# Alxaline/BraTS21

Hardware: AMD Instinct MI355X
Metric: train patches/sec (4x128^3, width-48) (higher is better)
Workload: dtype bf16; 1 GPU; equiunet width=48, batch=2/GPU of 4x128^3 synthetic patches, fwd + deep-supervision Dice + bwd + ranger (BASELINE.json configs[1]); global_batch=2, parallelism=dp1

## Files before the change

### brats21_amd/csrc/common.hpp

```cpp
#pragma once
#include <hip/hip_runtime.h>
#include <stdint.h>
#include <stdio.h>
#include <atomic>
#include <type_traits>
#include "../../include/brats_hip.h"

typedef uint16_t bf16_t;
#ifdef BRATS_FP16
typedef __attribute__((ext_vector_type(8))) _Float16 bf16x8;
typedef __attribute__((ext_vector_type(4))) _Float16 bf16x4;
#else
typedef __attribute__((ext_vector_type(8))) __bf16 bf16x8;
typedef __attribute__((ext_vector_type(4))) __bf16 bf16x4;
#endif
typedef __attribute__((ext_vector_type(4))) float f32x4;
typedef __attribute__((ext_vector_type(2))) float f32x2;
typedef __attribute__((ext_vector_type(4))) uint32_t u32x4;
typedef __attribute__((ext_vector_type(2))) uint32_t u32x2;

#define DEVI __device__ __forceinline__

#ifdef BRATS_FP16
DEVI float bf2f(bf16_t v) { return (float)__builtin_bit_cast(_Float16, v); }
// ... 190 lines not shown

static inline int ceil_div(int a, int b) { return (a + b - 1) / b; }

static inline int device_cus() {
  static int ncu = 0;
  if (!ncu) {
    int dev = 0;
    hipDeviceProp_t prop;
    ncu = (hipGetDevice(&dev) == hipSuccess && hipGetDeviceProperties(&prop, dev) == hipSuccess) ? prop.multiProcessorCount : 256;
  }
  return ncu;
}

template <typename T> struct type_tag { using type = T; };
template <typename F> static inline auto with_flag(bool on, F&& f) {
  if (on) return f(std::true_type{});
  return f(std::false_type{});
}
template <typename F> static inline auto with_storage(int dtype, F&& f) {
  if (dtype == BRATS_BF16) return f(type_tag<bf16_t>{});
  return f(type_tag<float>{});
}
template <typename F> static inline auto with_stream(int dtype, bool nt, F&& f) {
  return with_storage(dtype, [&](auto t) { return with_flag(nt, [&](auto n) { return f(t, n); }); });
}
template <typename F> static inline auto with_stream16(int dtype, bool nt, F&& f) {
  if (dtype != BRATS_BF16) return f(type_tag<float>{}, std::false_type{});
  return with_flag(nt, [&](auto n) { return f(type_tag<bf16_t>{}, n); });
}
template <typename F> static inline auto with_act_stream(int dtype, bool heavy, bool nt, F&& f) {
  if (heavy) return with_storage(dtype, [&](auto t) { return f(t, std::true_type{}, std::false_type{}); });
  return with_stream(dtype, nt, [&](auto t, auto n) { return f(t, std::false_type{}, n); });
}

static inline bool big_tensor(int dtype, size_t elems) { return stream_nt(elems * (dtype == BRATS_BF16 ? 2 : 4)); }
static inline bool big_tensor16(int dtype, size_t elems) { return dtype == BRATS_BF16 && stream_nt(elems * 2); }

static inline int vec_width(int dtype) { return dtype == BRATS_BF16 ? 8 : 4; }

static inline int stream_grid(size_t total, int block, int cap) {
  size_t b = (total + block - 1) / block;
  return (int)(b < 1 ? 1 : (b > (size_t)cap ? (size_t)cap : b));
}

struct Walk {
  int cv, vl;
  size_t blocks;
  unsigned grid(size_t cap) const { return (unsigned)(blocks < 1 ? 1 : (blocks > cap ? cap : blocks)); }
};
static inline Walk voxel_walk(int vw, int voxels, int C) {
  const int cv = C / vw, vl = 256 / cv;
  return Walk{cv, vl, ((size_t)voxels + (size_t)vl * 8 - 1) / ((size_t)vl * 8)};
}
```

### brats21_amd/csrc/gen_twin_dispatch.py

```python
#!/usr/bin/env python3
import re
import sys

BOTH = {"brats_conv3d_set_vs8", "brats_conv3d_set_kp", "brats_conv3d_set_wgrad_alltaps", "brats_conv3d_set_x3_wgrad_fused",
        "brats_upsample_bwd_set_fused"}
DATA = {"brats_conv3d_f8_fwd", "brats_conv3d_wgrad_f8", "brats_conv3d_pack_weights_multi"}

txt = re.sub(r"/\*.*?\*/", " ", open(sys.argv[1]).read(), flags=re.S)
protos = {}
for m in re.finditer(r"(const char\s*\*|size_t|int)\s+(brats_[a-z0-9_]+)\s*\(([^)]*)\)\s*;", txt):
    protos[m.group(2)] = (" ".join(m.group(1).split()), " ".join(m.group(3).split()))
names = []
for path in sys.argv[2:]:
    for m in re.finditer(r'extern "C" [a-z_ \*]+?BRATS_API\((brats_[a-z0-9_]+)\)\(', open(path).read()):
        names.append(m.group(1))
print("// GENERATED by gen_twin_dispatch.py from include/brats_hip.h -- do not edit")
print('#include "../../include/brats_hip.h"')
print('extern "C" {')
for n in names:
    if n not in protos:
        raise SystemExit(f"{n} is defined in a twinned translation unit but not declared in brats_hip.h")
    ret, args = protos[n]
    arglist = [] if args in ("", "void") else [a.strip() for a in args.split(",")]
    argnames = [re.search(r"([A-Za-z_][A-Za-z0-9_]*)$", a).group(1) for a in arglist]
    call = ", ".join(argnames)
    sig = args if arglist else "void"
    print(f"{ret} {n}_bf16({sig});")
    print(f"{ret} {n}_f16({sig});")
    if n in DATA:
        if n + "_f16" not in protos:
            raise SystemExit(f"{n}_f16 must be declared in brats_hip.h (16-bit data, no dtype argument)")
        print(f"{ret} {n}({sig}) {{ return {n}_bf16({call}); }}")
    elif n in BOTH:
        print(f"{ret} {n}({sig}) {{ {n}_f16({call}); return {n}_bf16({call}); }}")
    elif "dtype" in argnames:
        call16 = ", ".join("BRATS_BF16" if a == "dtype" else a for a in argnames)
        callx3 = ", ".join("BRATS_X3_BF16" if a == "dtype" else a for a in argnames)
        print(f"{ret} {n}({sig}) {{ return dtype == BRATS_F16 ? {n}_f16({call16}) : dtype == BRATS_X3_F16 ? {n}_f16({callx3}) : {n}_bf16({call}); }}")
    else:
        print(f"{ret} {n}({sig}) {{ return {n}_bf16({call}); }}")
print("}")
```

### brats21_amd/csrc/norm.hip

```cpp
#include "twin_begin.hpp"
#include "common.hpp"

#include "se.hpp"

constexpr int GN_MAX_SPLITS = 64;
__global__ void gn_chan_reduce_kernel(const float* __restrict__ stats, int tps, int C, double* __restrict__ part) {
  const int n = blockIdx.y, c0 = blockIdx.x * 16;
  const int cl = threadIdx.x & 15, tl = threadIdx.x >> 4;
  const int c = c0 + cl;
  const int per = (tps + gridDim.z - 1) / gridDim.z;
  const int t0 = blockIdx.z * per, t1 = min(tps, t0 + per);
  double s1 = 0.0, s2 = 0.0;
  if (c < C) {
    for (int t = t0 + tl; t < t1; t += 16) {
      const f32x2 v = *(const f32x2*)(stats + (((size_t)n * tps + t) * C + c) * 2);
      s1 += v[0];
      s2 += v[1];
    }
  }
  __shared__ double r1[256], r2[256];
  r1[threadIdx.x] = s1;
  r2[threadIdx.x] = s2;
  __syncthreads();
  for (int m = 128; m >= 16; m >>= 1) {
// ... 265 lines not shown
  if (!HEAVY && act == BRATS_ACT_RELU) run(std::true_type{});
  else run(std::false_type{});
  if (amax) record_absmax<T>(mx, amax);
}

extern "C" int BRATS_API(brats_affine_act_fwd)(const void* y, int ypitch, const float* scale_shift, void* z, int zpitch,
                                    int dtype, int act, float slope_value, const float* slope_dev, int N, int voxels, int C,
                                    float* amax, brats_stream_t s) {
  const SlopeArg slope{slope_value, slope_dev};
  const int vw = vec_width(dtype);
  if (!y || !z || !scale_shift || C % vw || ypitch % vw || zpitch % vw || C / vw > 256)
    BRATS_FAIL(BRATS_E_ARG, "affine_act_fwd: C and pitches must be multiples of %d (C <= %d)", vw, 256 * vw);
  const bool big = big_tensor(dtype, (size_t)N * voxels * C);
  dim3 grid(voxel_walk(vw, voxels, C).grid(big ? 8192 : 2048), N);
  with_act_stream(dtype, act > BRATS_ACT_LEAKY, big, [&](auto t, auto heavy, auto nt) {
    using T = typename decltype(t)::type;
    hipLaunchKernelGGL((affine_act_kernel<T, decltype(heavy)::value, decltype(nt)::value>), grid, dim3(256), 0, (hipStream_t)s, (const T*)y,
                       ypitch, scale_shift, (T*)z, zpitch, act, slope, voxels, C, (uint32_t*)amax);
  });
  BRATS_CHECK_LAUNCH();
  return 0;
}

template <typename T> struct Raw16;
template <> struct Raw16<bf16_t> {
  typedef u32x4 type;
  template <bool NT> static DEVI type load(const bf16_t* p) {
    if constexpr (NT) return __builtin_nontemporal_load((const u32x4*)p); else return *(const u32x4*)p;
  }
  static DEVI void unpack(const type& v, float* o) {
#pragma unroll
    for (int i = 0; i < 4; ++i) unpack2(v[i], o[2 * i], o[2 * i + 1]);
  }
};
template <> struct Raw16<float> {
  typedef f32x4 type;
  template <bool NT> static DEVI type load(const float* p) { return *(const f32x4*)p; }
  static DEVI void unpack(const type& v, float* o) { o[0] = v[0]; o[1] = v[1]; o[2] = v[2]; o[3] = v[3]; }
};

template <typename T, bool NT = false, bool AM = false>
__global__ void __launch_bounds__(256) affine_act_pool_kernel(const T* __restrict__ y, int ypitch, const float* __restrict__ scale_shift,
                                                              T* __restrict__ z, int zpitch, T* __restrict__ p, int ppitch, int act,
                                                              SlopeArg sl, int D, int H, int W, int C, int with_avg,
                                                              uint32_t* __restrict__ amax, uint8_t* __restrict__ argmax) {
  constexpr int VW = 16 / sizeof(T);
  typedef typename Raw16<T>::type raw_t;
  extern __shared__ __attribute__((aligned(16))) char pool_lds[];
  raw_t* xch = (raw_t*)pool_lds;
  const float slope = sl.p ? *sl.p : sl.v;
  const bool relu = act == BRATS_ACT_RELU;
  const int n = blockIdx.y;
  const int cv = C / VW;
  int xb = (blockDim.x / cv) & ~1;
  if (xb > W) xb = W;
  const int mycv = threadIdx.x % cv, myvl = threadIdx.x / cv, c0 = mycv * VW;
  const bool lane_on = myvl < xb;
  const int Do = D / 2, Ho = H / 2, Wo = W / 2;
  const int segs = (W + xb - 1) / xb;
  const size_t items = (size_t)Do * Ho * segs, voxels = (size_t)D * H * W;
  float sc[VW], sh[VW];
#pragma unroll
  for (int j = 0; j < VW; ++j) {
    sc[j] = lane_on ? scale_shift[((size_t)n * C + c0 + j) * 2] : 0.f;
    sh[j] = lane_on ? scale_shift[((size_t)n * C + c0 + j) * 2 + 1] : 0.f;
  }
  const T* yb = y + (size_t)n * voxels * ypitch + c0;
  T* zb = z + (size_t)n * voxels * zpitch + c0;
  T* pb = p + (size_t)n * Do * Ho * Wo * ppitch + c0;
  float amx = 0.f;
  int buf = 0;
  for (size_t item = blockIdx.x; item < items; item += gridDim.x, buf ^= 1) {
    const int seg = (int)(item % segs);
    const size_t rp = item / segs;
    const int yo = (int)(rp % Ho), zo = (int)(rp / Ho);
    const int x = seg * xb + myvl;
    const bool on = lane_on && x < W;
    raw_t mine[4];
    if (on) {
      raw_t raw[4];
      size_t vox[4];
#pragma unroll
      for (int k = 0; k < 4; ++k) {
        vox[k] = ((size_t)(2 * zo + (k >> 1)) * H + (2 * yo + (k & 1))) * W + x;
        raw[k] = Raw16<T>::template load<NT>(yb + vox[k] * ypitch);
      }
#pragma unroll
      for (int k = 0; k < 4; ++k) {
        float a[VW];
        Raw16<T>::unpack(raw[k], a);
#pragma unroll
        for (int j = 0; j < VW; ++j) {
          const float pre = a[j] * sc[j] + sh[j];
          const float neg = relu ? 0.f : pre * slope;
          a[j] = pre > 0.f ? pre : neg;
        }
        vstore<T, VW, NT>(zb + vox[k] * zpitch, a);
        if constexpr (std::is_same<T, float>::value) {
          mine[k] = raw_t{a[0], a[1], a[2], a[3]};
        } else {
#pragma unroll
          for (int q = 0; q < 4; ++q) mine[k][q] = pack2(a[2 * q], a[2 * q + 1]);
        }
        if (amax) {
          float r[VW];
          Raw16<T>::unpack(mine[k], r);
#pragma unroll
          for (int j = 0; j < VW; ++j) amx = __builtin_fmaxf(amx, __builtin_fabsf(r[j]));
        }
        xch[((size_t)buf * blockDim.x + threadIdx.x) * 4 + k] = mine[k];
      }
    }
    __syncthreads();
    if (on && !(myvl & 1)) {
      float mx[VW], sm[VW];
      int am[VW];
#pragma unroll
      for (int j = 0; j < VW; ++j) { mx[j] = -INFINITY; sm[j] = 0.f; am[j] = 0; }
#pragma unroll
      for (int k = 0; k < 4; ++k) {
        float a[VW], b[VW];
        Raw16<T>::unpack(mine[k], a);
        Raw16<T>::unpack(xch[((size_t)buf * blockDim.x + threadIdx.x + cv) * 4 + k], b);
#pragma unroll
        for (int j = 0; j < VW; ++j) {
          if constexpr (AM) {
            if (a[j] > mx[j] || a[j] != a[j]) { mx[j] = a[j]; am[j] = 2 * k; }
            if (b[j] > mx[j] || b[j] != b[j]) { mx[j] = b[j]; am[j] = 2 * k + 1; }
          } else {
            mx[j] = (a[j] > mx[j] || a[j] != a[j]) ? a[j] : mx[j];
            mx[j] = (b[j] > mx[j] || b[j] != b[j]) ? b[j] : mx[j];
          }
          sm[j] = (sm[j] + a[j]) + b[j];
        }
      }
      const size_t pvox = ((size_t)zo * Ho + yo) * Wo + (x >> 1);
      T* po = pb + pvox * ppitch;
      if constexpr (AM) {
        uint32_t w[VW / 4];
#pragma unroll
        for (int q = 0; q < VW / 4; ++q) w[q] = am[4 * q] | (am[4 * q + 1] << 8) | (am[4 * q + 2] << 16) | (am[4 * q + 3] << 24);
        uint32_t* ap = (uint32_t*)(argmax + ((size_t)n * Do * Ho * Wo + pvox) * C + c0);
#pragma unroll
        for (int q = 0; q < VW / 4; ++q) ap[q] = w[q];
      }
      Vec<T, VW>::store(po, mx);
      if (with_avg) {
#pragma unroll
        for (int j = 0; j < VW; ++j) sm[j] *= 0.125f;
        Vec<T, VW>::store(po + C, sm);
      }
    }
  }
  if (amax) record_absmax<T>(amx, amax);
}

extern "C" int BRATS_API(brats_affine_act_pool_fwd)(const void* y, int ypitch, const float* scale_shift, void* z, int zpitch, void* pooled,
                                         int ppitch, unsigned char* argmax, int dtype, int act, float slope_value,
                                         const float* slope_dev, int N, int D, int H, int W, int C, int with_avg, float* amax,
                                         brats_stream_t s) {
  const SlopeArg slope{slope_value, slope_dev};
  const int vw = vec_width(dtype);
  if (!y || !z || !pooled || !scale_shift || C % vw || ypitch % vw || zpitch % vw || ppitch % vw || C / vw > 256 || ((D | H | W) & 1))
    BRATS_FAIL(BRATS_E_ARG, "affine_act_pool_fwd: C / pitches multiples of %d (C <= %d), even spatial dims", vw, 256 * vw);
  if (act > BRATS_ACT_LEAKY) BRATS_FAIL(BRATS_E_UNSUPPORTED, "affine_act_pool_fwd: relu / leakyrelu only (act=%d)", act);
  int xb = (256 / (C / vw)) & ~1;
  if (xb < 2) BRATS_FAIL(BRATS_E_UNSUPPORTED, "affine_act_pool_fwd: C=%d leaves no pooling pair per block", C);
  if (xb > W) xb = W;
  const size_t items = (size_t)(D / 2) * (H / 2) * ((W + xb - 1) / xb);
  const bool big = big_tensor16(dtype, (size_t)N * D * H * W * C);
  dim3 grid(stream_grid(items, 1, big ? 8192 : 2048), N);
  const size_t lds = (size_t)2 * 256 * 4 * 16;
  with_stream16(dtype, big, [&](auto t, auto nt) {
    with_flag(argmax != nullptr, [&](auto am) {
      using T = typename decltype(t)::type;
      hipLaunchKernelGGL((affine_act_pool_kernel<T, decltype(nt)::value, decltype(am)::value>), grid, dim3(256), lds, (hipStream_t)s,
                         (const T*)y, ypitch, scale_shift, (T*)z, zpitch, (T*)pooled, ppitch, act, slope, D, H, W, C, with_avg,
                         (uint32_t*)amax, argmax);
    });
  });
  BRATS_CHECK_LAUNCH();
  return 0;
}

template <int VW, typename F>
DEVI void lane_reduce_plane(float* scr, const float* a, bool live, int myvl, int vl_n, int C, int c0, F&& put) {
  __syncthreads();
  if (live) {
#pragma unroll
    for (int j = 0; j < VW; ++j) scr[myvl * C + c0 + j] = a[j];
  }
  __syncthreads();
  for (int c = threadIdx.x; c < C; c += blockDim.x) {
    float t = 0.f;
    for (int l = 0; l < vl_n; ++l) t += scr[l * C + c];
    put(c, t);
  }
}

struct HeadFold {
  const float* dl = nullptr;
  const float* w = nullptr;
  float* hpart = nullptr;
  const void* dskip = nullptr;
  const void* dpool = nullptr;
  const uint8_t* argmax = nullptr;
  int dskip_pitch = 0, dpool_pitch = 0, D = 0, H = 0, W = 0;
  int with_avg = 0;
};
template <typename T, int VW>
DEVI void pool_dz(const HeadFold& hf, int n, size_t vox, int c0, int C, typename Raw16<T>::type& skr, typename Raw16<T>::type& dpr,
                  typename Raw16<T>::type& avr, uint32_t (&aw)[VW / 4], int& kk) {
  const int x = (int)(vox % hf.W);
  const size_t t = vox / hf.W;
  const int yy = (int)(t % hf.H), z = (int)(t / hf.H);
  const size_t pvox = (((size_t)n * (hf.D / 2) + (z >> 1)) * (hf.H / 2) + (yy >> 1)) * (hf.W / 2) + (x >> 1);
  kk = ((z & 1) << 2) | ((yy & 1) << 1) | (x & 1);
  skr = Raw16<T>::template load<false>((const T*)hf.dskip + ((size_t)n * hf.D * hf.H * hf.W + vox) * hf.dskip_pitch + c0);
  dpr = Raw16<T>::template load<false>((const T*)hf.dpool + pvox * hf.dpool_pitch + c0);
  if (hf.with_avg) avr = Raw16<T>::template load<false>((const T*)hf.dpool + pvox * hf.dpool_pitch + C + c0);
  else avr = dpr;
#pragma unroll
  for (int q = 0; q < VW / 4; ++q) aw[q] = ((const uint32_t*)(hf.argmax + pvox * C + c0))[q];
}
// ... 1486 lines not shown
```

### brats21_amd/csrc/pool_up.hip

```cpp
#include "twin_begin.hpp"
#include "common.hpp"

constexpr int POOL_MAX_BLOCKS = 8192;

template <typename T>
__global__ void maxpool2_fwd_kernel(const T* __restrict__ x, int xpitch, T* __restrict__ y, int ypitch, int N, int C,
                                    int D, int H, int W, int with_avg, uint8_t* __restrict__ argmax) {
  constexpr int VW = 16 / sizeof(T);
  const int cv = C / VW, Do = D / 2, Ho = H / 2, Wo = W / 2;
  const size_t total = (size_t)N * Do * Ho * Wo * cv;
  for (size_t it = (size_t)blockIdx.x * blockDim.x + threadIdx.x; it < total; it += (size_t)gridDim.x * blockDim.x) {
    const int c0 = (int)(it % cv) * VW;
    size_t v = it / cv;
    const int xo = v % Wo; v /= Wo;
    const int yo = v % Ho; v /= Ho;
    const int zo = v % Do;
    const int n = (int)(v / Do);
    float mx[VW], sm[VW];
    int am[VW];
#pragma unroll
    for (int j = 0; j < VW; ++j) { mx[j] = -INFINITY; sm[j] = 0.f; am[j] = 0; }
#pragma unroll
    for (int k = 0; k < 8; ++k) {
      const int z = 2 * zo + (k >> 2), yy = 2 * yo + ((k >> 1) & 1), xx = 2 * xo + (k & 1);
// ... 284 lines not shown
#pragma unroll
    for (int a = 0; a < 2; ++a)
#pragma unroll
      for (int b = 0; b < 4; ++b)
#pragma unroll
        for (int j = 0; j < V2; ++j) o[a][b][j] = f2{0.f, 0.f};
#pragma unroll
    for (int pz = 0; pz < 3; ++pz) {
      const int zi = zb + pz < D ? zb + pz : D - 1;
      f2 t[4][V2];
#pragma unroll
      for (int b = 0; b < 4; ++b)
#pragma unroll
        for (int j = 0; j < V2; ++j) t[b][j] = f2{0.f, 0.f};
#pragma unroll
      for (int r = 0; r < 4; ++r) {
        const int yi = yb + r < H ? yb + r : H - 1;
        float v0[VW], v1[VW];
        if constexpr (LDSX) {
          const T* row = (const T*)up_lds + (size_t)(pz * 4 + r) * W * C + c0;
          Vec<T, VW>::load(row + (size_t)lx.i0 * C, v0);
          Vec<T, VW>::load(row + (size_t)lx.i1 * C, v1);
        } else {
          const T* row = xb + (size_t)(zi * H + yi) * W * xpitch + c0;
          Vec<T, VW>::load(row + (size_t)lx.i0 * xpitch, v0);
          Vec<T, VW>::load(row + (size_t)lx.i1 * xpitch, v1);
        }
#pragma unroll
        for (int j = 0; j < V2; ++j) {
          const f2 xl = fma2(lx.w1, f2{v1[2 * j], v1[2 * j + 1]}, lx.w0 * f2{v0[2 * j], v0[2 * j + 1]});
#pragma unroll
          for (int b = 0; b < 4; ++b) t[b][j] = fma2(wy[b][r], xl, t[b][j]);
        }
      }
#pragma unroll
      for (int a = 0; a < 2; ++a)
#pragma unroll
        for (int b = 0; b < 4; ++b)
#pragma unroll
          for (int j = 0; j < V2; ++j) o[a][b][j] = fma2(wz[a][pz], t[b][j], o[a][b][j]);
    }
#pragma unroll
    for (int a = 0; a < 2; ++a)
#pragma unroll
      for (int b = 0; b < 4; ++b) {
        float of[VW];
#pragma unroll
        for (int j = 0; j < V2; ++j) { of[2 * j] = o[a][b][j][0]; of[2 * j + 1] = o[a][b][j][1]; }
        vstore<T, VW, NT>(yb_ + ((size_t)((zo0 + a) * Ho + yo0 + b) * Wo + xo) * ypitch + c0, of);
      }
  }
}

extern "C" int BRATS_API(brats_upsample_fwd)(const void* x, int xpitch, void* y, int ypitch, int dtype, int N, int C, int D, int H,
                                  int W, int scale, brats_stream_t s) {
  const int vw = vec_width(dtype);
  if (!x || !y || C % vw || xpitch % vw || ypitch % vw || scale < 1)
    BRATS_FAIL(BRATS_E_ARG, "upsample_fwd: C/pitch must be multiples of %d", vw);
  const size_t rows = (size_t)N * D * scale * H * scale;
  const unsigned grid = (unsigned)(rows > 65536 ? 65536 : rows);
  const float sd = ac_scale(D, D * scale), sh = ac_scale(H, H * scale), sw = ac_scale(W, W * scale);
  if (scale == 2 && H % 2 == 0 && N <= 65535 && D <= 65535) {
    const dim3 g2(H / 2, D, N);
    const size_t ldsx = (size_t)12 * W * C * 2;
    const bool big = big_tensor16(dtype, (size_t)N * D * H * W * 8 * C);
    auto go = [&](auto t, auto nt, auto in_lds) {
      using T = typename decltype(t)::type;
      constexpr bool LDSX = decltype(in_lds)::value;
      hipLaunchKernelGGL((upsample2_fwd_kernel<T, decltype(nt)::value, LDSX>), g2, dim3(256), LDSX ? ldsx : 0, (hipStream_t)s, (const T*)x,
                         xpitch, (T*)y, ypitch, C, D, H, W, sd, sh, sw);
    };
    if (dtype == BRATS_BF16 && ldsx <= 80 * 1024) {
      static std::atomic<uint64_t> attr_a{0}, attr_b{0};
      BRATS_ENSURE_LDS_ATTR((upsample2_fwd_kernel<bf16_t, true, true>), 80 * 1024, attr_a);
      BRATS_ENSURE_LDS_ATTR((upsample2_fwd_kernel<bf16_t, false, true>), 80 * 1024, attr_b);
      with_flag(big, [&](auto nt) { go(type_tag<bf16_t>{}, nt, std::true_type{}); });
    } else {
      with_stream16(dtype, big, [&](auto t, auto nt) { go(t, nt, std::false_type{}); });
    }
    BRATS_CHECK_LAUNCH();
    return 0;
  }
  with_storage(dtype, [&](auto t) {
    using T = typename decltype(t)::type;
    hipLaunchKernelGGL(upsample_fwd_kernel<T>, dim3(grid), dim3(256), 0, (hipStream_t)s, (const T*)x, xpitch, (T*)y, ypitch, N, C, D, H, W,
                       scale, sd, sh, sw);
  });
  BRATS_CHECK_LAUNCH();
  return 0;
}

template <typename T, int VW>
DEVI void add_stored(float* acc, const T* addp) {
  float b[VW];
  if constexpr (VW == 1) b[0] = to_f<T>(addp[0]);
  else Vec<T, VW>::load(addp, b);
#pragma unroll
  for (int j = 0; j < VW; ++j) acc[j] = to_f<T>(from_f<T>(acc[j])) + b[j];
}

template <typename TI, typename TO, int VW, bool ADD = false>
__global__ void lerp_adjoint_kernel(const TI* __restrict__ in, int in_pitch, TO* __restrict__ out, int out_pitch,
                                    size_t outer, int Lout , int Lin , size_t inner_vox, int C,
                                    float scale, const TO* __restrict__ add = nullptr ,
                                    int add_pitch = 0) {
  const int cv = C / VW;
  const size_t total = outer * Lin * inner_vox * cv;
  const float inv = scale > 0.f ? 1.f / scale : 0.f;
  for (size_t it = (size_t)blockIdx.x * blockDim.x + threadIdx.x; it < total; it += (size_t)gridDim.x * blockDim.x) {
    const int c0 = (int)(it % cv) * VW;
    size_t v = it / cv;
    const size_t iv = v % inner_vox; v /= inner_vox;
    const int i = (int)(v % Lin);
    const size_t o = v / Lin;
    int lo = (int)floorf((float)(i - 1) * inv) - 1, hi = (int)ceilf((float)(i + 1) * inv) + 1;
    if (scale <= 0.f) { lo = 0; hi = Lout - 1; }
    lo = lo < 0 ? 0 : lo;
    hi = hi > Lout - 1 ? Lout - 1 : hi;
    float acc[VW];
#pragma unroll
    for (int j = 0; j < VW; ++j) acc[j] = 0.f;
    for (int l = lo; l <= hi; ++l) {
      const Lerp c = lerp_coef(l, Lin, scale);
      float w = 0.f;
      if (c.i0 == i) w += c.w0;
// ... 430 lines not shown
```

### brats21_amd/ops.py

```python
import contextlib
import weakref

import numpy as np
import torch

from . import _lib
from ._lib import ACT_LEAKY, ACT_NONE, ACT_RELU, BF16, F16, F32, PACK_DGRAD, PACK_FWD, X3_BF16, X3_F16

ACTS = {"none": ACT_NONE, "relu": ACT_RELU, "leakyrelu": ACT_LEAKY, "elu": _lib.ACT_ELU, "swish": _lib.ACT_SWISH,
        "mish": _lib.ACT_MISH}


class KernelTimer:

    def __init__(self):
        self.records = {}

    def span(self, key):
        return _Span(self, key)

    def summary(self):
        torch.cuda.synchronize()
        out = {}
        for key, evs in self.records.items():
# ... 747 lines not shown
def prelu_slope_grad(dz, y, scale_shift):
    dzp, c, dzpitch = _desc(dz)
    yp, _, ypitch = _desc(y)
    n, d, h, w, _ = y.shape
    ws = torch.empty(_lib.lib().brats_prelu_ws_floats(n), dtype=torch.float32, device=y.device)
    out = torch.empty(1, dtype=torch.float32, device=y.device)
    _lib.check(_lib.lib().brats_prelu_slope_grad(dzp, dzpitch, yp, ypitch, scale_shift.data_ptr(), ws.data_ptr(), out.data_ptr(),
                                                 _code(y.dtype), n, d * h * w, c, _stream()), "prelu_slope_grad")
    return out


def maxpool2(x, with_avg=False, out=None, want_argmax=False):
    ptr, c, p = _desc(x)
    n, d, h, w, _ = x.shape
    co = 2 * c if with_avg else c
    if out is None:
        out = new_act(n, d // 2, h // 2, w // 2, co, x.dtype, x.device)
    optr, oc, op = _desc(out)
    idx = torch.empty((n, d // 2, h // 2, w // 2, c), dtype=torch.uint8, device=x.device) if want_argmax else None
    _lib.check(_lib.lib().brats_maxpool2_fwd(ptr, p, optr, op, idx.data_ptr() if idx is not None else None, _code(x.dtype), n, c, d,
                                             h, w, int(with_avg), _stream()), "maxpool2_fwd")
    if idx is not None:
        x._pool_argmax = idx
    return out


def maxpool2_bwd(x, dy, dx_skip=None, with_avg=False):
    ptr, c, p = _desc(x)
    dptr, _, dp = _desc(dy)
    n, d, h, w, _ = x.shape
    dx = new_act(n, d, h, w, c, x.dtype, x.device)
    sptr, sp = (None, 0)
    if dx_skip is not None:
        sptr, _, sp = _desc(dx_skip)
    idx = getattr(x, "_pool_argmax", None)
    if idx is not None:
        _lib.check(_lib.lib().brats_maxpool2_bwd_idx(idx.data_ptr(), dptr, dp, sptr, sp, dx.data_ptr(), c, _code(x.dtype), n, c,
                                                     d, h, w, int(with_avg), _stream()), "maxpool2_bwd_idx")
        return dx
    _lib.check(_lib.lib().brats_maxpool2_bwd(ptr, p, None, 0, dptr, dp, sptr, sp, dx.data_ptr(), c, _code(x.dtype), n, c,
                                             d, h, w, int(with_avg), _stream()), "maxpool2_bwd")
    return dx


def upsample(x, scale=2, out=None):
    ptr, c, p = _desc(x)
    n, d, h, w, _ = x.shape
    if out is None:
        out = new_act(n, d * scale, h * scale, w * scale, c, x.dtype, x.device)
    optr, oc, op = _desc(out)
    _lib.check(_lib.lib().brats_upsample_fwd(ptr, p, optr, op, _code(x.dtype), n, c, d, h, w, scale, _stream()),
               "upsample_fwd")
    return out


def set_upsample_bwd_fused(mode):
    return _lib.lib().brats_upsample_bwd_set_fused(mode)


def upsample_bwd(dy, scale=2, add=None, out=None):
    dptr, c, dp = _desc(dy)
    n, do, ho, wo, _ = dy.shape
    d, h, w = do // scale, ho // scale, wo // scale
    code = _code(dy.dtype)
    ws = torch.empty(_lib.lib().brats_upsample_bwd_ws_bytes(code, n, c, d, h, w, scale), dtype=torch.uint8, device=dy.device)
    dx = new_act(n, d, h, w, c, dy.dtype, dy.device) if out is None else out
    xptr, xc, xp = _desc(dx)
    if tuple(dx.shape) != (n, d, h, w, c) or dx.dtype != dy.dtype:
        raise ValueError(f"upsample_bwd: out {tuple(dx.shape)} {dx.dtype} does not match {(n, d, h, w, c)} {dy.dtype}")
    if add is None:
        _lib.check(_lib.lib().brats_upsample_bwd(dptr, dp, xptr, xp, ws.data_ptr(), code, n, c, d, h, w, scale, _stream()), "upsample_bwd")
        return dx
    if tuple(add.shape) != (n, d, h, w, c) or add.dtype != dy.dtype:
        raise ValueError(f"upsample_bwd: addend {tuple(add.shape)} {add.dtype} does not match {(n, d, h, w, c)} {dy.dtype}")
    aptr, _, ap = _desc(add)
    _lib.check(_lib.lib().brats_upsample_bwd_add(dptr, dp, aptr, ap, xptr, xp, ws.data_ptr(), code, n, c, d, h, w, scale, _stream()),
               "upsample_bwd_add")
    return dx


def upsample_nearest(x, scale=2, out=None):
    ptr, c, p = _desc(x)
    n, d, h, w, _ = x.shape
    if out is None:
        out = new_act(n, d * scale, h * scale, w * scale, c, x.dtype, x.device)
    optr, oc, op = _desc(out)
    if tuple(out.shape) != (n, d * scale, h * scale, w * scale, c) or out.dtype != x.dtype:
        raise ValueError(f"upsample_nearest: out {tuple(out.shape)} {out.dtype} does not match {(n, d * scale, h * scale, w * scale, c)} {x.dtype}")
    _lib.check(_lib.lib().brats_upsample_nearest_fwd(ptr, p, optr, op, _code(x.dtype), n, c, d, h, w, scale, _stream()),
               "upsample_nearest_fwd")
    return out


def upsample_nearest_bwd(dy, scale=2, add=None, out=None):
    dptr, c, dp = _desc(dy)
    n, do, ho, wo, _ = dy.shape
    if do % scale or ho % scale or wo % scale:
        raise ValueError(f"upsample_nearest_bwd: the extent {(do, ho, wo)} is no multiple of the scale {scale}")
    d, h, w = do // scale, ho // scale, wo // scale
    dx = new_act(n, d, h, w, c, dy.dtype, dy.device) if out is None else out
    xptr, xc, xp = _desc(dx)
    if tuple(dx.shape) != (n, d, h, w, c) or dx.dtype != dy.dtype:
        raise ValueError(f"upsample_nearest_bwd: out {tuple(dx.shape)} {dx.dtype} does not match {(n, d, h, w, c)} {dy.dtype}")
    aptr, ap = None, 0
    if add is not None:
        if tuple(add.shape) != (n, d, h, w, c) or add.dtype != dy.dtype:
# ... 685 lines not shown
```

### include/brats_hip.h

```cpp
#ifndef BRATS_HIP_H
#define BRATS_HIP_H
#include <stddef.h>
#include <stdint.h>

#ifdef __cplusplus
extern "C" {
#endif

typedef void* brats_stream_t;

enum { BRATS_F32 = 0, BRATS_BF16 = 1, BRATS_F16 = 2, BRATS_X3_BF16 = 3, BRATS_X3_F16 = 4 };
enum { BRATS_E_ARG = -1, BRATS_E_UNSUPPORTED = -2, BRATS_E_HIP = -3 };
enum { BRATS_ACT_NONE = 0, BRATS_ACT_RELU = 1, BRATS_ACT_LEAKY = 2, BRATS_ACT_ELU = 3, BRATS_ACT_SWISH = 4, BRATS_ACT_MISH = 5 };

#define BRATS_ABI_VERSION 7
int brats_abi_version(void);
const char* brats_last_error(void);

int brats_dropout(const void* x, int xpitch, void* out, int opitch, int dtype, size_t voxels, int C, float p,
                  const void* state, int unit, brats_stream_t s);

int brats_ncdhw_to_ndhwc(const float* src, void* dst, int dtype, int N, int C, int cpad, int dst_pitch,
                         int D, int H, int W, brats_stream_t s);
int brats_ndhwc_to_ncdhw(const void* src, int src_pitch, float* dst, int dtype, int N, int C,
// ... 132 lines not shown
                            int xpitch, const float* mean_rstd, const float* gamma, const float* beta, void* dx, int dxpitch,
                            float* red, float* dgamma, float* dbeta, const double* chan_sums, float* dconvbias, int dtype,
                            int N, int voxels, int C, int groups, float* amax, brats_stream_t s);
int brats_se_fwd(const float* chansum, float inv_vox, const float* w1, const float* b1, const float* w2, const float* b2,
                 float* gate1p , float* hidden , int N, int C, int Ch, brats_stream_t s);
int brats_se_bwd(const float* dgate, const float* chansum, float inv_vox, const float* hidden, const float* gate1p,
                 const float* w1, const float* w2, float* gadd , float* dw1, float* db1, float* dw2, float* db2,
                 int N, int C, int Ch, brats_stream_t s);
int brats_evonorm_se_bwd(const void* dout, int dopitch, const void* x, int xpitch, const float* mean_rstd, const float* gamma,
                         const float* beta, void* dx, int dxpitch, float* ws, float* dgamma, float* dbeta,
                         const double* chan_sums, float* dconvbias, const float* se_chansum, const float* hidden,
                         const float* gate1p, const float* w1, const float* w2, float* gadd, float* dw1, float* db1,
                         float* dw2, float* db2, int Ch,
                         const float* dlogits ,
                         const float* hw , int K, float* hws ,
                         float* dhw , float* dhb ,
                         int dtype, int N, int voxels, int C, int groups, float* amax, brats_stream_t s);
int brats_evonorm_se_bwd_pool(const void* dskip, int dskip_pitch, const void* dpool, int dpool_pitch, const unsigned char* argmax,
                              int with_avg, int D, int H, int W, const void* x, int xpitch, const float* mean_rstd,
                              const float* gamma, const float* beta, void* dx, int dxpitch, float* ws, float* dgamma,
                              float* dbeta, const double* chan_sums, float* dconvbias, const float* se_chansum,
                              const float* hidden, const float* gate1p, const float* w1, const float* w2, float* gadd,
                              float* dw1, float* db1, float* dw2, float* db2, int Ch, int dtype, int N, int C, int groups,
                              float* amax, brats_stream_t s);
int brats_evonorm_se_fwd(const void* x, int xpitch, const float* mean_rstd, const float* gamma, const float* beta,
                         const float* w1, const float* b1, const float* w2, const float* b2, void* out, int opitch,
                         float* ws, float* chansum_out, float* gate1p, float* hidden, int Ch, int dtype, int N, int voxels,
                         int C, int groups, float* amax ,
                         brats_stream_t s);
int brats_channel_dot(const void* a, int apitch, const void* b , int bpitch, float* out ,
                      int dtype, int N, int voxels, int C, brats_stream_t s);
int brats_channel_scale(const void* a, int apitch, const float* scale , const float* add ,
                        void* dst, int dpitch, int dtype, int N, int voxels, int C,
                        float* amax , brats_stream_t s);
typedef struct { const void* x; const void* w; int xpitch, cin, ksize, dil; } brats_dconv_term;
typedef struct { brats_dconv_term term[4]; int nterms, rows; const float* bias; void* y; int ypitch, reserved; } brats_dconv_job;
size_t brats_dconv_packed_bytes(int dtype, int ksize, int kdim, int rows);
int brats_dconv_pack_weights(const float* w, void* packed, int dtype, int mode, int ksize, int cout_w, int cin_w,
                             int cin_off, int cin_cnt, brats_stream_t s);
int brats_dconv_run(const brats_dconv_job* jobs, int njobs, int dtype, int N, int D, int H, int W, brats_stream_t s);

int brats_maxpool2_fwd(const void* x, int xpitch, void* y, int ypitch,
                       unsigned char* argmax ,
                       int dtype, int N, int C, int D, int H, int W, int with_avg, brats_stream_t s);
int brats_maxpool2_bwd(const void* x, int xpitch, const void* y, int ypitch, const void* dy, int dypitch,
                       const void* dx_skip, int dxskip_pitch, void* dx, int dxpitch, int dtype,
                       int N, int C, int D, int H, int W, int with_avg, brats_stream_t s);
int brats_maxpool2_bwd_idx(const unsigned char* argmax, const void* dy, int dypitch, const void* dx_skip ,
                           int dxskip_pitch, void* dx, int dxpitch, int dtype, int N, int C, int D, int H, int W,
                           int with_avg, brats_stream_t s);

int brats_upsample_fwd(const void* x, int xpitch, void* y, int ypitch, int dtype, int N, int C,
                       int D, int H, int W, int scale, brats_stream_t s);
size_t brats_upsample_bwd_ws_bytes(int dtype, int N, int C, int D, int H, int W, int scale);
int brats_upsample_bwd(const void* dy, int dypitch, void* dx, int dxpitch, void* tmp, int dtype,
                       int N, int C, int D, int H, int W, int scale, brats_stream_t s);
int brats_upsample_bwd_add(const void* dy, int dypitch, const void* add, int addpitch, void* dx, int dxpitch, void* tmp,
                           int dtype, int N, int C, int D, int H, int W, int scale, brats_stream_t s);
int brats_upsample_bwd_set_fused(int mode);

int brats_upsample_nearest_fwd(const void* x, int xpitch, void* y, int ypitch, int dtype, int N, int C,
                               int D, int H, int W, int scale, brats_stream_t s);
int brats_upsample_nearest_bwd(const void* dy, int dypitch, const void* add , int addpitch, void* dx, int dxpitch,
                               int dtype, int N, int C, int D, int H, int W, int scale, brats_stream_t s);
int brats_planes_nearest_fwd(const float* low, float* out, int planes, int D, int H, int W, int scale, brats_stream_t s);
int brats_planes_nearest_bwd(const float* dout, float* dlow, int planes, int D, int H, int W, int scale, brats_stream_t s);

size_t brats_conv3d_narrow_packed_bytes(int C, int K);
int brats_conv3d_narrow_pack(const float* w, float* packed, int mode, int cout_w, int cin_w, brats_stream_t s);
int brats_conv3d_narrow_fwd(const void* x, int C, int xpitch, const float* packed_w, const float* bias, const float* add, float* out,
                            int dtype, int K, int N, int D, int H, int W, brats_stream_t s);

int brats_head_fwd(const void* x, int xpitch, const float* w , const float* b, float* lowres ,
                   float* out , int dtype, int N, int C, int K,
                   int D, int H, int W, int scale, brats_stream_t s);
int brats_gn_head_fwd(const void* y, int ypitch, const float* scale_shift, int act, float slope, const float* w ,
                      const float* b, float* out, int dtype, int N, int C, int K, int voxels, brats_stream_t s);
int brats_evonorm_head_fwd(const void* y, int ypitch, const float* scale_shift, const float* w , const float* b,
                           float* out, int dtype, int N, int C, int K, int voxels, brats_stream_t s);
size_t brats_head_bwd_ws_bytes(int N, int C, int K, int D, int H, int W, int scale);
int brats_head_bwd(const void* x, int xpitch, const float* w, const float* dout, float* ws,
                   void* dx, int dxpitch, float* dw, float* db, int dtype, int N, int C, int K,
                   int D, int H, int W, int scale, brats_stream_t s);

int brats_sw_gather(const float* src, float* dst, const int* windows, int B, int C, int D, int H, int W,
                    int rd, int rh, int rw, int pad_z, int pad_y, int pad_x, float cval, int pad_mode, brats_stream_t s);
int brats_sw_accumulate(const float* prob, const float* importance, float* out, float* count, int K,
                        int Dp, int Hp, int Wp, int rd, int rh, int rw, int n, int z0, int y0, int x0,
                        brats_stream_t s);
int brats_sw_accumulate_multi(const float* prob, const float* importance, float* out, float* count, const int* windows,
                              int B, int NB, int K, int Dp, int Hp, int Wp, int rd, int rh, int rw, brats_stream_t s);
int brats_sw_finalize(const float* out, const float* count, float* dst, int NK, int Dp, int Hp, int Wp,
                      int D, int H, int W, int pad_z, int pad_y, int pad_x, brats_stream_t s);

int brats_spatial_signed_perm(const float* src, float* dst, int planes, int s0, int s1, int s2,
                              int p0, int p1, int p2, int f0, int f1, int f2, int mode, brats_stream_t s);

size_t brats_dice_ws_floats(int N, int K);
int brats_dice_stats(const float* logits, const float* target, float* sums , float* ws, int N, int K,
                     size_t voxels, brats_stream_t s);
int brats_dice_grad(const float* logits, const float* target, const float* coef ,
                    float* dlogits, int N, int K, size_t voxels, brats_stream_t s);
size_t brats_dice_multi_ws_floats(int H, int N, int K);
int brats_dice_stats_multi(const float* const* heads, int H, const float* target, float* ws, int N, int K, size_t voxels,
                           brats_stream_t s);
int brats_dice_finish(const float* ws, int H, int N, int K, size_t voxels, float eps, int jaccard, float* sums, float* coef,
// ... 177 lines not shown
```

Before: 144.1 patches/s.

## Add z-walking trilinear upsample kernel and prefetch next item in fused pool

Adds a bf16 trilinear upsample-forward kernel that walks output z-planes within a block, keeping a rolling three-plane LDS window and prefetching the next input plane into registers while the current planes are computed. It is selected by default when shapes fit, and a new set_form knob can force or disable it. The fused affine+act+maxpool kernel now flattens work items across rows rather than per-row segments, and software-pipelines the next item's global loads ahead of the barrier. It also drops the larger grid cap for big tensors. The aim is to hide load latency and cut redundant input reads, at the cost of register pressure and extra code paths.

```diff
diff --git a/brats21_amd/csrc/common.hpp b/brats21_amd/csrc/common.hpp
--- a/brats21_amd/csrc/common.hpp
+++ b/brats21_amd/csrc/common.hpp
@@ -266,3 +266,14 @@
   const int cv = C / vw, vl = 256 / cv;
   return Walk{cv, vl, ((size_t)voxels + (size_t)vl * 8 - 1) / ((size_t)vl * 8)};
 }
+
+struct PoolWalk {
+  int xb;
+  size_t total, items;
+};
+__host__ __device__ static inline PoolWalk pool_walk(int threads, int cv, int D, int H, int W) {
+  int xb = (threads / cv) & ~1;
+  if (xb > W) xb = W;
+  const size_t total = (size_t)(D / 2) * (H / 2) * W;
+  return PoolWalk{xb, total, xb < 2 ? 0 : (total + xb - 1) / xb};
+}
diff --git a/brats21_amd/csrc/gen_twin_dispatch.py b/brats21_amd/csrc/gen_twin_dispatch.py
--- a/brats21_amd/csrc/gen_twin_dispatch.py
+++ b/brats21_amd/csrc/gen_twin_dispatch.py
@@ -3,7 +3,7 @@
 import sys
 
 BOTH = {"brats_conv3d_set_vs8", "brats_conv3d_set_kp", "brats_conv3d_set_wgrad_alltaps", "brats_conv3d_set_x3_wgrad_fused",
-        "brats_upsample_bwd_set_fused"}
+        "brats_upsample_bwd_set_fused", "brats_upsample_fwd_set_form"}
 DATA = {"brats_conv3d_f8_fwd", "brats_conv3d_wgrad_f8", "brats_conv3d_pack_weights_multi"}
 
 txt = re.sub(r"/\*.*?\*/", " ", open(sys.argv[1]).read(), flags=re.S)
diff --git a/brats21_amd/csrc/norm.hip b/brats21_amd/csrc/norm.hip
--- a/brats21_amd/csrc/norm.hip
+++ b/brats21_amd/csrc/norm.hip
@@ -341,13 +341,12 @@
   const bool relu = act == BRATS_ACT_RELU;
   const int n = blockIdx.y;
   const int cv = C / VW;
-  int xb = (blockDim.x / cv) & ~1;
-  if (xb > W) xb = W;
+  const PoolWalk pw = pool_walk(blockDim.x, cv, D, H, W);
+  const int xb = pw.xb;
   const int mycv = threadIdx.x % cv, myvl = threadIdx.x / cv, c0 = mycv * VW;
   const bool lane_on = myvl < xb;
   const int Do = D / 2, Ho = H / 2, Wo = W / 2;
-  const int segs = (W + xb - 1) / xb;
-  const size_t items = (size_t)Do * Ho * segs, voxels = (size_t)D * H * W;
+  const size_t rows = (size_t)Do * Ho, voxels = (size_t)D * H * W;
   float sc[VW], sh[VW];
 #pragma unroll
   for (int j = 0; j < VW; ++j) {
@@ -359,21 +358,39 @@
   T* pb = p + (size_t)n * Do * Ho * Wo * ppitch + c0;
   float amx = 0.f;
   int buf = 0;
-  for (size_t item = blockIdx.x; item < items; item += gridDim.x, buf ^= 1) {
-    const int seg = (int)(item % segs);
-    const size_t rp = item / segs;
-    const int yo = (int)(rp % Ho), zo = (int)(rp / Ho);
-    const int x = seg * xb + myvl;
-    const bool on = lane_on && x < W;
+  struct Pos { int x, yo, zo; size_t rp; bool on; };
+  auto locate = [&](size_t item) {
+    const size_t rp0 = item * xb / W, zo0 = rp0 / Ho;
+    Pos q{(int)(item * xb - rp0 * W) + myvl, (int)(rp0 - zo0 * Ho), (int)zo0, rp0, false};
+    if (q.x >= W) {
+      q.x -= W, ++q.rp;
+      if (++q.yo == Ho) q.yo = 0, ++q.zo;
+    }
+    q.on = lane_on && q.rp < rows;
+    return q;
+  };
+  auto voxel = [&](const Pos& q, int k) { return ((size_t)(2 * q.zo + (k >> 1)) * H + (2 * q.yo + (k & 1))) * W + q.x; };
+  auto load4 = [&](const Pos& q, raw_t* raw) {
+    if (q.on) {
+#pragma unroll
+      for (int k = 0; k < 4; ++k) raw[k] = Raw16<T>::template load<NT>(yb + voxel(q, k) * ypitch);
+    }
+  };
+  Pos cur{0, 0, 0, 0, false};
+  raw_t raw[4];
+  if (blockIdx.x < pw.items) {
+    cur = locate(blockIdx.x);
+    load4(cur, raw);
+  }
+  for (size_t item = blockIdx.x; item < pw.items; item += gridDim.x, buf ^= 1) {
+    const bool on = cur.on;
+    const int x = cur.x;
+    const size_t rp = cur.rp;
     raw_t mine[4];
     if (on) {
-      raw_t raw[4];
       size_t vox[4];
 #pragma unroll
-      for (int k = 0; k < 4; ++k) {
-        vox[k] = ((size_t)(2 * zo + (k >> 1)) * H + (2 * yo + (k & 1))) * W + x;
-        raw[k] = Raw16<T>::template load<NT>(yb + vox[k] * ypitch);
-      }
+      for (int k = 0; k < 4; ++k) vox[k] = voxel(cur, k);
 #pragma unroll
       for (int k = 0; k < 4; ++k) {
         float a[VW];
@@ -399,6 +416,12 @@
         }
         xch[((size_t)buf * blockDim.x + threadIdx.x) * 4 + k] = mine[k];
       }
+    }
+    Pos nxt{0, 0, 0, 0, false};
+    raw_t rawn[4] = {};
+    if (item + gridDim.x < pw.items) {
+      nxt = locate(item + gridDim.x);
+      load4(nxt, rawn);
     }
     __syncthreads();
     if (on && !(myvl & 1)) {
@@ -423,7 +446,7 @@
           sm[j] = (sm[j] + a[j]) + b[j];
         }
       }
-      const size_t pvox = ((size_t)zo * Ho + yo) * Wo + (x >> 1);
+      const size_t pvox = rp * Wo + (x >> 1);
       T* po = pb + pvox * ppitch;
       if constexpr (AM) {
         uint32_t w[VW / 4];
@@ -440,6 +463,9 @@
         Vec<T, VW>::store(po + C, sm);
       }
     }
+    cur = nxt;
+#pragma unroll
+    for (int k = 0; k < 4; ++k) raw[k] = rawn[k];
   }
   if (amax) record_absmax<T>(amx, amax);
 }
@@ -453,12 +479,10 @@
   if (!y || !z || !pooled || !scale_shift || C % vw || ypitch % vw || zpitch % vw || ppitch % vw || C / vw > 256 || ((D | H | W) & 1))
     BRATS_FAIL(BRATS_E_ARG, "affine_act_pool_fwd: C / pitches multiples of %d (C <= %d), even spatial dims", vw, 256 * vw);
   if (act > BRATS_ACT_LEAKY) BRATS_FAIL(BRATS_E_UNSUPPORTED, "affine_act_pool_fwd: relu / leakyrelu only (act=%d)", act);
-  int xb = (256 / (C / vw)) & ~1;
-  if (xb < 2) BRATS_FAIL(BRATS_E_UNSUPPORTED, "affine_act_pool_fwd: C=%d leaves no pooling pair per block", C);
-  if (xb > W) xb = W;
-  const size_t items = (size_t)(D / 2) * (H / 2) * ((W + xb - 1) / xb);
+  const PoolWalk pw = pool_walk(256, C / vw, D, H, W);
+  if (pw.xb < 2) BRATS_FAIL(BRATS_E_UNSUPPORTED, "affine_act_pool_fwd: C=%d leaves no pooling pair per block", C);
   const bool big = big_tensor16(dtype, (size_t)N * D * H * W * C);
-  dim3 grid(stream_grid(items, 1, big ? 8192 : 2048), N);
+  dim3 grid(stream_grid(pw.items, 1, 2048), N);
   const size_t lds = (size_t)2 * 256 * 4 * 16;
   with_stream16(dtype, big, [&](auto t, auto nt) {
     with_flag(argmax != nullptr, [&](auto am) {
diff --git a/brats21_amd/csrc/pool_up.hip b/brats21_amd/csrc/pool_up.hip
--- a/brats21_amd/csrc/pool_up.hip
+++ b/brats21_amd/csrc/pool_up.hip
@@ -360,6 +360,151 @@
   }
 }
 
+constexpr int UPW_PF = 7;
+template <bool NT>
+__global__ void __launch_bounds__(256, 2) upsample2_fwd_walk_kernel(const bf16_t* __restrict__ x, int xpitch, bf16_t* __restrict__ y, int ypitch,
+                                                                    int C, int D, int H, int W, int cd, float sd, float sh, float sw) {
+  typedef bf16_t T;
+  constexpr int VW = 8, V2 = VW / 2;
+  extern __shared__ __attribute__((aligned(16))) char up_lds[];
+  const int cv = C / VW, Ho = 2 * H, Wo = 2 * W;
+  const int yq = blockIdx.x, n = blockIdx.z;
+  const int zp0 = blockIdx.y * cd, zp1 = zp0 + cd < D ? zp0 + cd : D;
+  const int yo0 = 4 * yq;
+  Lerp ly[4];
+#pragma unroll
+  for (int b = 0; b < 4; ++b) ly[b] = lerp_coef(yo0 + b, H, sh);
+  const int yb = ly[0].i0;
+  float wy[4][4];
+#pragma unroll
+  for (int b = 0; b < 4; ++b)
+#pragma unroll
+    for (int r = 0; r < 4; ++r) wy[b][r] = (ly[b].i0 == yb + r ? ly[b].w0 : 0.f) + (ly[b].i1 == yb + r ? ly[b].w1 : 0.f);
+  const T* xb = x + (size_t)n * D * H * W * xpitch;
+  T* yb_ = y + (size_t)n * 2 * D * Ho * Wo * ypitch;
+  const int row_pieces = W * cv, plane_pieces = 4 * row_pieces;
+  auto piece = [&](int p, int q) {
+    const int r = q / row_pieces, w = q % row_pieces;
+    const int yi = yb + r < H ? yb + r : H - 1;
+    return *(const u32x4*)(xb + ((size_t)(p * H + yi) * W + w / cv) * xpitch + (w % cv) * VW);
+  };
+  auto slot = [&](int p) { return up_lds + (size_t)(p % 3) * plane_pieces * 16; };
+  auto stage = [&](int p) {
+    for (int q = threadIdx.x; q < plane_pieces; q += blockDim.x) *(u32x4*)(slot(p) + (size_t)q * 16) = piece(p, q);
+  };
+  int top;
+  {
+    const int zb = lerp_coef(2 * zp0, D, sd).i0;
+    top = zb + 2 < D ? zb + 2 : D - 1;
+    for (int p = zb; p <= top; ++p) stage(p);
+  }
+  __syncthreads();
+  typedef __attribute__((ext_vector_type(2))) float f2;
+  auto fma2 = [](float w, f2 v, f2 acc) { return __builtin_elementwise_fma(f2{w, w}, v, acc); };
+  for (int zp = zp0; zp < zp1; ++zp) {
+    const int zo0 = 2 * zp;
+    Lerp lz[2];
+#pragma unroll
+    for (int a = 0; a < 2; ++a) lz[a] = lerp_coef(zo0 + a, D, sd);
+    const int zb = lz[0].i0;
+    float wz[2][3];
+#pragma unroll
+    for (int a = 0; a < 2; ++a)
+#pragma unroll
+      for (int pz = 0; pz < 3; ++pz) wz[a][pz] = (lz[a].i0 == zb + pz ? lz[a].w0 : 0.f) + (lz[a].i1 == zb + pz ? lz[a].w1 : 0.f);
+    int zbn = zb, ntop = top;
+    if (zp + 1 < zp1) {
+      zbn = lerp_coef(zo0 + 2, D, sd).i0;
+      ntop = zbn + 2 < D ? zbn + 2 : D - 1;
+    }
+    const bool adv = ntop > top;
+    u32x4 pf[UPW_PF];
+    if (adv) {
+#pragma unroll
+      for (int k = 0; k < UPW_PF; ++k) {
+        const int q = threadIdx.x + k * 256;
+        if (q < plane_pieces) pf[k] = piece(top + 1, q);
+      }
+    }
+    const char* pl[3];
+#pragma unroll
+    for (int pz = 0; pz < 3; ++pz) pl[pz] = slot(zb + pz < D ? zb + pz : D - 1);
+    for (int it = threadIdx.x; it < Wo * cv; it += blockDim.x) {
+      const int xo = it / cv, c0 = (it % cv) * VW;
+      const Lerp lx = lerp_coef(xo, W, sw);
+      f2 o[2][4][V2];
+#pragma unroll
+      for (int a = 0; a < 2; ++a)
+#pragma unroll
+        for (int b = 0; b < 4; ++b)
+#pragma unroll
+          for (int j = 0; j < V2; ++j) o[a][b][j] = f2{0.f, 0.f};
+#pragma unroll
+      for (int pz = 0; pz < 3; ++pz) {
+        f2 t[4][V2];
+#pragma unroll
+        for (int b = 0; b < 4; ++b)
+#pragma unroll
+          for (int j = 0; j < V2; ++j) t[b][j] = f2{0.f, 0.f};
+#pragma unroll
+        for (int r = 0; r < 4; ++r) {
+          float v0[VW], v1[VW];
+          const T* row = (const T*)pl[pz] + (size_t)r * W * C + c0;
+          Vec<T, VW>::load(row + (size_t)lx.i0 * C, v0);
+          Vec<T, VW>::load(row + (size_t)lx.i1 * C, v1);
+#pragma unroll
+          for (int j = 0; j < V2; ++j) {
+            const f2 xl = fma2(lx.w1, f2{v1[2 * j], v1[2 * j + 1]}, lx.w0 * f2{v0[2 * j], v0[2 * j + 1]});
+#pragma unroll
+            for (int b = 0; b < 4; ++b) t[b][j] = fma2(wy[b][r], xl, t[b][j]);
+          }
+        }
+#pragma unroll
+        for (int a = 0; a < 2; ++a)
+#pragma unroll
+          for (int b = 0; b < 4; ++b)
+#pragma unroll
+            for (int j = 0; j < V2; ++j) o[a][b][j] = fma2(wz[a][pz], t[b][j], o[a][b][j]);
+      }
+#pragma unroll
+      for (int a = 0; a < 2; ++a)
+#pragma unroll
+        for (int b = 0; b < 4; ++b) {
+          float of[VW];
+#pragma unroll
+          for (int j = 0; j < V2; ++j) { of[2 * j] = o[a][b][j][0]; of[2 * j + 1] = o[a][b][j][1]; }
+          vstore<T, VW, NT>(yb_ + ((size_t)((zo0 + a) * Ho + yo0 + b) * Wo + xo) * ypitch + c0, of);
+        }
+    }
+    if (adv) {
+      __syncthreads();
+#pragma unroll
+      for (int k = 0; k < UPW_PF; ++k) {
+        const int q = threadIdx.x + k * 256;
+        if (q < plane_pieces) *(u32x4*)(slot(top + 1) + (size_t)q * 16) = pf[k];
+      }
+      for (int p = top + 2 > zbn ? top + 2 : zbn; p <= ntop; ++p) stage(p);
+      top = ntop;
+      __syncthreads();
+    }
+  }
+}
+
+static int g_upsample_fwd_form = -1;
+extern "C" int BRATS_API(brats_upsample_fwd_set_form)(int mode) {
+  const int old = g_upsample_fwd_form;
+  g_upsample_fwd_form = mode < 0 ? -1 : (mode ? 1 : 0);
+  return old;
+}
+static int upsample_fwd_walk_cd(int dtype, int N, int C, int D, int H, int W, int ypitch, bool big) {
+  if (g_upsample_fwd_form == 0 || dtype != BRATS_BF16 || (size_t)12 * W * C * 2 > 80 * 1024 || 4 * W * (C / 8) > UPW_PF * 256) return 0;
+  const size_t per_z = (size_t)N * (H / 2);
+  int cd = 16;
+  while (cd > 2 && per_z * ceil_div(D, cd) < 1024) cd /= 2;
+  if (g_upsample_fwd_form < 0 && (per_z * ceil_div(D, cd) < 512 || (big && ypitch != C))) return 0;
+  return cd;
+}
+
 extern "C" int BRATS_API(brats_upsample_fwd)(const void* x, int xpitch, void* y, int ypitch, int dtype, int N, int C, int D, int H,
                                   int W, int scale, brats_stream_t s) {
   const int vw = vec_width(dtype);
@@ -378,7 +523,15 @@
       hipLaunchKernelGGL((upsample2_fwd_kernel<T, decltype(nt)::value, LDSX>), g2, dim3(256), LDSX ? ldsx : 0, (hipStream_t)s, (const T*)x,
                          xpitch, (T*)y, ypitch, C, D, H, W, sd, sh, sw);
     };
-    if (dtype == BRATS_BF16 && ldsx <= 80 * 1024) {
+    if (const int cd = upsample_fwd_walk_cd(dtype, N, C, D, H, W, ypitch, big)) {
+      static std::atomic<uint64_t> attr_wa{0}, attr_wb{0};
+      BRATS_ENSURE_LDS_ATTR((upsample2_fwd_walk_kernel<true>), 80 * 1024, attr_wa);
+      BRATS_ENSURE_LDS_ATTR((upsample2_fwd_walk_kernel<false>), 80 * 1024, attr_wb);
+      with_flag(big, [&](auto nt) {
+        hipLaunchKernelGGL((upsample2_fwd_walk_kernel<decltype(nt)::value>), dim3(H / 2, ceil_div(D, cd), N), dim3(256), ldsx, (hipStream_t)s,
+                           (const bf16_t*)x, xpitch, (bf16_t*)y, ypitch, C, D, H, W, cd, sd, sh, sw);
+      });
+    } else if (dtype == BRATS_BF16 && ldsx <= 80 * 1024) {
       static std::atomic<uint64_t> attr_a{0}, attr_b{0};
       BRATS_ENSURE_LDS_ATTR((upsample2_fwd_kernel<bf16_t, true, true>), 80 * 1024, attr_a);
       BRATS_ENSURE_LDS_ATTR((upsample2_fwd_kernel<bf16_t, false, true>), 80 * 1024, attr_b);
diff --git a/brats21_amd/ops.py b/brats21_amd/ops.py
--- a/brats21_amd/ops.py
+++ b/brats21_amd/ops.py
@@ -823,6 +823,10 @@
     _lib.check(_lib.lib().brats_upsample_fwd(ptr, p, optr, op, _code(x.dtype), n, c, d, h, w, scale, _stream()),
                "upsample_fwd")
     return out
+
+
+def set_upsample_fwd_form(mode):
+    return _lib.lib().brats_upsample_fwd_set_form(mode)
 
 
 def set_upsample_bwd_fused(mode):
diff --git a/include/brats_hip.h b/include/brats_hip.h
--- a/include/brats_hip.h
+++ b/include/brats_hip.h
@@ -208,6 +208,7 @@
 
 int brats_upsample_fwd(const void* x, int xpitch, void* y, int ypitch, int dtype, int N, int C,
                        int D, int H, int W, int scale, brats_stream_t s);
+int brats_upsample_fwd_set_form(int mode);
 size_t brats_upsample_bwd_ws_bytes(int dtype, int N, int C, int D, int H, int W, int scale);
 int brats_upsample_bwd(const void* dy, int dypitch, void* dx, int dxpitch, void* tmp, int dtype,
                        int N, int C, int D, int H, int W, int scale, brats_stream_t s);
```

New measurement: 145.1 patches/s (median of 6 runs). Within noise of the previous version (+0.7%).
